# xaynetwork/xaynet

Measured on AMD Instinct MI355X. Metric: masked updates aggregated/sec (25M-param f32 model, PET round: aggregate+all-reduce+unmask), higher is better.
Workload: dtype f32; 1 GPU; model=pet-masked-aggregation-25M, global_batch=1250, seq_len=25000000, parallelism=client-sharded dp1 + rccl all-reduce, mask_config=Prime/F32/B0/M6 (7-byte limbs)

## Files before the change

### xaynet_amd/csrc/gpu/hip_bindings.cpp

```cpp
#include <pybind11/pybind11.h>

#include <pybind11/stl.h>

#include <cmath>
#include <cstring>
#include <stdexcept>
#include <string>
#include <utility>
#include <vector>

#include "kernels.h"

namespace py = pybind11;

struct Limbs {
    xhip_limbs v;
    int n;

    bool is_zero() const { return n == 1 && v.w[0] == 0; }
};

static Limbs parse_limbs(const std::string& dec) {
    if (dec.empty()) throw std::runtime_error("bad decimal");
    Limbs r{{{0, 0, 0, 0, 0}}, 1};
// ... 165 lines not shown

        std::vector<uint32_t> staging(10 * S);
        std::memcpy(staging.data(), seeds.data(), 32 * S);
        std::memcpy(staging.data() + 8 * S, start_words.data(), 8 * S);
        key_.reserve(10 * S, "alloc keys");
        check(hipMemcpy(key_.get(), staging.data(), 40 * S, hipMemcpyHostToDevice), "seed H2D");

        const Plan pl = plan(order, prng_nbytes, len, attempts);
        if (S == 1 || !pl.batchable) {
            uint64_t launched = 0;
            for (uint64_t s = 0; s < S; ++s)
                launched += finish(key_.get() + 8 * s, start_words[s], out_lo + s * seed_stride,
                                   out_hi ? out_hi + s * seed_stride : nullptr, len, order,
                                   prng_nbytes, 0, 0, attempts);
            return launched;
        }

        const uint64_t cand_stride = pl.wgs * 256 * pl.apt;
        const uint32_t counts_stride = uint32_t(pl.wgs);
        cand_lo_.reserve(S * cand_stride, "alloc cand");
        if (order.n == 2) cand_hi_.reserve(S * cand_stride, "alloc cand_hi");
        counts_.reserve(S * counts_stride, "alloc counts");
        total_.reserve(S, "alloc totals");
        check(xhip_k1_expand_batch(
                  key_.get(), reinterpret_cast<const uint64_t*>(key_.get() + 8 * S), uint32_t(S),
                  pl.n_att, pl.wpd, prng_nbytes, order.v.w[0], order.v.w[1], cand_lo_.get(),
                  order.n == 2 ? cand_hi_.get() : nullptr, cand_stride, counts_.get(),
                  counts_stride, total_.get(), pl.apt, out_lo, out_hi, seed_stride, len),
              "k1_expand_batch");
        std::vector<uint64_t> totals(S);
        check(hipMemcpy(totals.data(), total_.get(), 8 * S, hipMemcpyDeviceToHost),
              "totals D2H");
        uint64_t launched = S * pl.n_att;
        for (uint64_t s = 0; s < S; ++s) {
            if (totals[s] >= len) continue;
            launched += finish(key_.get() + 8 * s, start_words[s], out_lo + s * seed_stride,
                               out_hi ? out_hi + s * seed_stride : nullptr, len, order,
                               prng_nbytes, totals[s], pl.n_att, 0) -
                        pl.n_att;
        }
        return launched;
    }

  private:
    uint64_t finish(const uint32_t* key_dev, uint64_t start_word, uint64_t* out_lo,
                    uint64_t* out_hi, uint64_t len, const Limbs& order, int prng_nbytes,
                    uint64_t filled, uint64_t attempt, uint64_t first_attempts) {
        const int L = order.n;
        total_.reserve(1, "alloc total");
        while (filled < len) {
            const Plan pl = plan(order, prng_nbytes, len - filled, first_attempts);
            first_attempts = 0;
            const uint64_t n_att = pl.n_att;
            uint64_t max_wgs = pl.wgs + 2;
            cand_lo_.reserve(L > 2 ? L * n_att : n_att, "alloc cand");
            if (L == 2) cand_hi_.reserve(n_att, "alloc cand_hi");
            uint64_t* cand_hi = L > 2 ? cand_lo_.get() + n_att : cand_hi_.get();
            counts_.reserve(max_wgs, "alloc counts");
            scan_tmp_.reserve(max_wgs / 1024 + 2, "alloc scan tmp");

            uint32_t n_wgs = 0;
            check(xhip_k1_candidates_limbs(key_dev, start_word, attempt, n_att, pl.wpd,
                                           prng_nbytes, order.v, cand_lo_.get(), cand_hi,
                                           counts_.get(), pl.apt, &n_wgs),
                  "k1_candidates");
            check(xhip_k1_scan_hier(counts_.get(), n_wgs, scan_tmp_.get(), total_.get()),
                  "k1_scan");
            check(xhip_k1_scatter_compact_limbs(cand_lo_.get(), cand_hi, counts_.get(),
                                                total_.get(), n_wgs, pl.apt, filled, out_lo,
                                                out_hi, len, order.v),
                  "k1_scatter_compact");
            uint64_t round_accepted = 0;
            check(hipMemcpy(&round_accepted, total_.get(), 8, hipMemcpyDeviceToHost),
                  "total D2H");
            filled += round_accepted;
            if (filled > len) filled = len;
            attempt += n_att;
            if (round_accepted == 0 && n_att > 0 && pl.p <= 0.0)
                throw std::runtime_error("expand: zero acceptance");
        }
        return attempt;
    }

    static constexpr uint64_t kMaxAttemptsPerLaunch = uint64_t(1) << 22;

    DeviceBuffer<uint64_t> cand_lo_;
    DeviceBuffer<uint64_t> cand_hi_;
    DeviceBuffer<uint32_t> counts_;
    DeviceBuffer<uint32_t> scan_tmp_;
    DeviceBuffer<uint64_t> total_;
    DeviceBuffer<uint32_t> key_;
};

PYBIND11_MODULE(_hip, m) {
    m.doc() = "xaynet_amd MI355X (gfx950) kernels: mask expand, aggregate, unmask";
    const auto nogil = py::call_guard<py::gil_scoped_release>();

    m.def("device_count", []() {
        int n = 0;
        hipError_t e = hipGetDeviceCount(&n);
        return e == hipSuccess ? n : 0;
    });
    m.def("synchronize", []() { check(hipDeviceSynchronize(), "sync"); });

    m.def("host_register", [](uintptr_t ptr, size_t size) {
        check(hipHostRegister(reinterpret_cast<void*>(ptr), size, hipHostRegisterDefault),
              "hipHostRegister");
    });
    m.def("host_unregister", [](uintptr_t ptr) {
        check(hipHostUnregister(reinterpret_cast<void*>(ptr)), "hipHostUnregister");
    });

    py::class_<MaskExpander>(m, "MaskExpander")
        .def(py::init<>())
        .def(
            "expand",
            [](MaskExpander& self, const std::string& seed, uintptr_t out_lo, uintptr_t out_hi,
               uint64_t len, const std::string& order, int prng_nbytes, py::object start_word,
               uint64_t seed_stride, uint64_t attempts) {
                std::vector<uint64_t> words;
                if (py::isinstance<py::int_>(start_word))
                    words.push_back(start_word.cast<uint64_t>());
                else
                    words = start_word.cast<std::vector<uint64_t>>();
                py::gil_scoped_release release;
                return self.expand(seed, out_lo, out_hi, len, order, prng_nbytes, words,
                                   seed_stride, attempts);
            },
            py::arg("seed"), py::arg("out_lo"), py::arg("out_hi"), py::arg("len"),
            py::arg("order"), py::arg("prng_nbytes"), py::arg("start_word"), py::kw_only(),
            py::arg("seed_stride") = 0, py::arg("attempts") = 0)
        .def_static("_batch_size", &MaskExpander::batch_size, py::arg("len"), py::arg("order"),
                    py::arg("prng_nbytes"), py::arg("budget_bytes"));

    m.def(
        "aggregate_batch",
        [](uintptr_t acc, uintptr_t updates, uint64_t stride, uint32_t n_updates, uint64_t len,
           int bpn, int ept) {
            check(xhip_k3_aggregate(u64p(acc), u8p(updates), stride, n_updates, len, bpn, ept),
                  "k3_aggregate");
        },
        py::arg("acc"), py::arg("updates"), py::arg("stride"), py::arg("n_updates"),
        py::arg("len"), py::arg("bpn"), py::arg("ept") = 0, nogil);

    m.def(
        "_k3_tile_plan",
        [](uint64_t len, int bpn, uint64_t stride) {
            XhipK3TilePlan p;
            xhip_k3_tile_plan(len, bpn, stride, &p);
            py::dict d;
            d["tile_elems"] = p.tile_elems;
            d["depth"] = p.depth;
            d["waves"] = p.waves;
            d["n_tiles"] = p.n_tiles;
            d["rem_start"] = p.rem_start;
            d["max_byte"] = p.max_byte;
            return d;
        },
        py::arg("len"), py::arg("bpn"), py::arg("stride"));

    m.def(
        "_read_ceiling",
        [](uintptr_t src, uint64_t bytes, bool nontemporal, uintptr_t sink) {
            check(xhip_read_ceiling(u8p(src), bytes, nontemporal,
                                    reinterpret_cast<uint32_t*>(sink)),
                  "read_ceiling");
        },
        py::arg("src"), py::arg("bytes"), py::arg("nontemporal"), py::arg("sink"), nogil);

    m.def(
        "_model_encode",
        [](uintptr_t src, int dtype, uint64_t len, uintptr_t work, uintptr_t out,
           uint64_t out_bytes) -> uint64_t {
            if (dtype < 0 || dtype > 3) throw py::value_error("dtype must be 0..3");
            if (len > (uint64_t(1) << 32))
                throw py::value_error("a model has at most 2^32 weights");
            if (len == 0) return 9;
            py::gil_scoped_release release;
            void* w = reinterpret_cast<void*>(src);
            void* ws = reinterpret_cast<void*>(work);
            check(xhip_k7_model_count(w, dtype, len, ws), "k7_model_count");
            uint64_t words = 0;
            check(hipMemcpy(&words, ws, sizeof words, hipMemcpyDeviceToHost), "k7 total");
            const uint64_t body = 9 + 4 * words;
            if (out_bytes >= 3 + body)
                check(xhip_k7_model_emit(w, dtype, len, ws, u8p(out), out_bytes),
                      "k7_model_emit");
            return body;
        },
        py::arg("src"), py::arg("dtype"), py::arg("len"), py::arg("work"), py::arg("out"),
        py::arg("out_bytes"));

    m.def(
        "_model_plan",
        [](uint64_t len) {
            XhipK7Plan p;
            xhip_k7_plan(len, &p);
            py::dict d;
            d["block_elems"] = p.block_elems;
            d["blocks"] = p.blocks;
            d["scan_levels"] = p.scan_levels;
            d["tile_blocks"] = p.tile_blocks;
            d["tiles"] = p.tiles;
            d["work_bytes"] = p.work_bytes;
            return d;
        },
        py::arg("len"));

    m.def(
        "unmask",
        [](uintptr_t planes, uintptr_t mask_lo, uintptr_t mask_hi, uintptr_t out, uint64_t len,
           int n_planes, const std::string& order, const std::string& exp_shift,
           double n_add_shift, double scalar_sum, int dtype, int digit_bits,
           const std::string& offset, const std::string& divisor) {
            Limbs o = parse_order(order, mask_hi), e = parse_limbs(exp_shift);
            Limbs off = parse_optional(offset), div = parse_optional(divisor);
            check_digit_bits(o, digit_bits);
            if (off.is_zero()) {
                if (o.n > 2)
                    throw py::value_error("orders >= 2^128 are Bmax configs: unmask needs "
                                          "their exact offset");
                if (e.n > 2) throw py::value_error("exp_shift >= 2^128 needs the exact offset");
                if (!div.is_zero()) throw py::value_error("divisor goes with an offset");
            } else if (off.n > o.n) {
                throw py::value_error("the exact offset must be below the order");
            }
            if (div.n > 1) throw py::value_error("divisor must be below 2^64");
            const double scale = double(1.0L / (limbs_to_ld(e) * (long double)scalar_sum));
            check(xhip_k4_unmask_limbs(u64p(planes), u64p(mask_lo), u64p(mask_hi), dtype,
                                       reinterpret_cast<void*>(out), len, n_planes, digit_bits,
                                       o.v, e.v, n_add_shift, scalar_sum, off.v, div.v.w[0],
                                       scale),
                  "k4_unmask");
        },
        py::arg("planes"), py::arg("mask_lo"), py::arg("mask_hi"), py::arg("out"),
        py::arg("len"), py::arg("n_planes"), py::arg("order"), py::arg("exp_shift"),
        py::arg("n_add_shift"), py::arg("scalar_sum"), py::arg("dtype") = 0,
        py::arg("digit_bits") = 32, py::arg("offset") = "", py::arg("divisor") = "", nogil);

    m.def(
        "unmask_values",
        [](uintptr_t vals, uintptr_t mask_lo, uintptr_t mask_hi, uintptr_t out, uint64_t len,
           const std::string& order, const std::string& exp_shift, double n_add_shift,
           double scalar_sum, int dtype, const std::string& offset,
           const std::string& divisor) {
            Limbs o = parse_order(order, mask_hi), e = parse_limbs(exp_shift);
            Limbs off = parse_optional(offset), div = parse_optional(divisor);
            if (o.n > 1 || e.n > 1) throw py::value_error("unmask_values covers u64 orders");
            if (off.n > 1 || div.n > 1)
                throw py::value_error("offset and divisor must be below 2^64");
            if (off.is_zero() && !div.is_zero())
                throw py::value_error("divisor goes with an offset");
            check(xhip_k4_unmask_values(u64p(vals), u64p(mask_lo), dtype,
                                        reinterpret_cast<void*>(out), len, o.v.w[0], e.v.w[0],
                                        n_add_shift, scalar_sum, off.v.w[0], div.v.w[0]),
                  "k4_unmask_values");
        },
        py::arg("vals"), py::arg("mask_lo"), py::arg("mask_hi"), py::arg("out"), py::arg("len"),
        py::arg("order"), py::arg("exp_shift"), py::arg("n_add_shift"), py::arg("scalar_sum"),
        py::arg("dtype") = 0, py::arg("offset") = "", py::arg("divisor") = "", nogil);

    m.def(
        "canonicalize",
        [](uintptr_t planes, uintptr_t out_lo, uintptr_t out_hi, uint64_t len, int n_planes,
           const std::string& order, int digit_bits) {
            Limbs o = parse_order(order, out_hi);
            check_digit_bits(o, digit_bits);
            check(xhip_k2_canonicalize_limbs(u64p(planes), u64p(out_lo), u64p(out_hi), len,
                                             n_planes, digit_bits, o.v),
                  "k2_canonicalize");
        },
        py::arg("planes"), py::arg("out_lo"), py::arg("out_hi"), py::arg("len"),
        py::arg("n_planes"), py::arg("order"), py::arg("digit_bits") = 32, nogil);

    m.def(
        "add_to_planes",
        [](uintptr_t planes, uintptr_t lo, uintptr_t hi, uint64_t len, int n_planes,
           const std::string& order, int digit_bits, uint32_t rows, uint64_t row_stride) {
            Limbs o = parse_order(order, hi);
            check_digit_bits(o, digit_bits);
            if (rows < 1 || rows > XHIP_K1_MAX_BATCH)
                throw py::value_error("rows must be in 1..65535");
            if (rows > 1 && (row_stride == 0 || row_stride < len))
                throw py::value_error("several rows need row_stride, the u64 elements between "
                                      "them (at least len)");
            check(xhip_add_rows_to_planes_limbs(u64p(planes), u64p(lo), u64p(hi), len, n_planes,
                                                digit_bits, o.v, rows, row_stride),
                  "add_to_planes");
        },
        py::arg("planes"), py::arg("lo"), py::arg("hi"), py::arg("len"), py::arg("n_planes"),
        py::arg("order"), py::arg("digit_bits") = 32, py::kw_only(), py::arg("rows") = 1,
        py::arg("row_stride") = 0, nogil);

    m.def(
        "recode_planes",
        [](uintptr_t acc, uintptr_t out, uint64_t len, int n_digits, const std::string& order,
           int k, int digit_bits) {
            Limbs o = parse_limbs(order);
            if (o.n == 1) throw py::value_error("recode_planes covers wide (>= 2^64) orders");
            check(xhip_k2_recode_planes_limbs(u64p(acc), u64p(out), len, n_digits, o.v, k,
                                              digit_bits),
                  "k2_recode_planes");
        },
        py::arg("acc"), py::arg("out"), py::arg("len"), py::arg("n_digits"), py::arg("order"),
        py::arg("k"), py::arg("digit_bits"), nogil);

// ... 94 lines not shown
```

### xaynet_amd/csrc/gpu/kernels.h

```cpp
#pragma once

#include <hip/hip_runtime.h>

#include <cstdint>

#include "limbs.h"

extern "C" {

hipError_t xhip_k1_candidates(const uint32_t* key8_dev, uint64_t start_word,
                              uint64_t first_attempt, uint64_t n_attempts, int words_per_draw,
                              int nbytes, uint64_t order_lo, uint64_t order_hi,
                              uint64_t* cand_lo, uint64_t* cand_hi, uint32_t* wg_counts,
                              int attempts_per_thread, uint32_t* n_wgs_out);
#define XHIP_K1_SCAN_ONE_WG 2048
#define XHIP_K1_MAX_BATCH 65535
hipError_t xhip_k1_scan_hier(uint32_t* wg_counts, uint32_t n, uint32_t* blk_tmp,
                             uint64_t* total_dev);
hipError_t xhip_k1_scatter_compact(const uint64_t* cand_lo, const uint64_t* cand_hi,
                                   const uint32_t* wg_offsets, const uint64_t* total_dev,
                                   uint32_t n_wgs, int apt, uint64_t out_base, uint64_t* out_lo,
                                   uint64_t* out_hi, uint64_t out_len);
hipError_t xhip_k1_expand_batch(const uint32_t* keys_dev, const uint64_t* start_words_dev,
                                uint32_t n_seeds, uint64_t n_attempts, int words_per_draw,
                                int nbytes, uint64_t order_lo, uint64_t order_hi,
                                uint64_t* cand_lo, uint64_t* cand_hi, uint64_t cand_stride,
                                uint32_t* wg_counts, uint32_t counts_stride,
                                uint64_t* totals_dev, int apt, uint64_t* out_lo,
                                uint64_t* out_hi, uint64_t out_stride, uint64_t out_len);

hipError_t xhip_k3_aggregate(uint64_t* acc, const uint8_t* updates, uint64_t stride,
                             uint32_t n_updates, uint64_t len, int bpn, int ept);

struct XhipK3TilePlan {
    uint32_t tile_elems, depth, waves;
    uint64_t n_tiles, rem_start;
    int64_t max_byte;
};
void xhip_k3_tile_plan(uint64_t len, int bpn, uint64_t stride, XhipK3TilePlan* plan);

hipError_t xhip_read_ceiling(const uint8_t* src, uint64_t bytes, bool nontemporal,
                             uint32_t* sink);

hipError_t xhip_k4_unmask(const uint64_t* planes, const uint64_t* mask_lo,
                          const uint64_t* mask_hi, int dtype, void* out, uint64_t len,
                          int n_planes, int digit_bits, uint64_t order_lo, uint64_t order_hi,
                          uint64_t exp_lo, uint64_t exp_hi, double n_add_shift,
                          double scalar_sum);
hipError_t xhip_k4_unmask_values(const uint64_t* vals, const uint64_t* mask, int dtype,
                                 void* out, uint64_t len, uint64_t order, uint64_t exp_shift,
                                 double n_add_shift, double scalar_sum, uint64_t offset,
                                 uint64_t divisor);
hipError_t xhip_k2_canonicalize(const uint64_t* planes, uint64_t* out_lo, uint64_t* out_hi,
                                uint64_t len, int n_planes, int digit_bits, uint64_t order_lo,
                                uint64_t order_hi);
hipError_t xhip_add_to_planes(uint64_t* planes, const uint64_t* lo, const uint64_t* hi,
                              uint64_t len, int n_planes, int digit_bits);
hipError_t xhip_k2_recode_planes(const uint64_t* acc, uint64_t* out, uint64_t len, int n_digits,
                                 uint64_t order_lo, uint64_t order_hi, int k, int digit_bits);
hipError_t xhip_k2_mod_add(uint64_t* a_lo, uint64_t* a_hi, const uint64_t* b_lo,
                           const uint64_t* b_hi, uint64_t len, uint64_t order_lo,
                           uint64_t order_hi);

hipError_t xhip_k5_mask_pack(const uint64_t* mask_lo, const uint64_t* mask_hi, uint8_t* out,
                             uint64_t len, int bpn, uint64_t order_lo, uint64_t order_hi,
                             uint64_t participant, double scalar, double add_shift,
                             uint64_t exp_lo, uint64_t exp_hi);
hipError_t xhip_k5_mask_weights(const void* w, int dtype, const uint64_t* mask_lo,
                                const uint64_t* mask_hi, uint8_t* out, uint64_t len, int bpn,
                                uint64_t order_lo, uint64_t order_hi, double scalar,
                                double add_shift, uint64_t exp_lo, uint64_t exp_hi);

hipError_t xhip_k6_unpack(const uint8_t* in, uint64_t* out_lo, uint64_t* out_hi, uint64_t len,
                          int bpn);
hipError_t xhip_k6_pack(const uint64_t* in_lo, const uint64_t* in_hi, uint8_t* out, uint64_t len,
                        int bpn);

#define XHIP_K7_SCAN_ONE_WG 4096
struct XhipK7Plan {
    uint32_t block_elems, scan_levels, tile_blocks;
    uint64_t blocks, tiles, work_bytes;
};
void xhip_k7_plan(uint64_t len, XhipK7Plan* plan);
hipError_t xhip_k7_model_count(const void* w, int dtype, uint64_t len, void* work);
hipError_t xhip_k7_model_emit(const void* w, int dtype, uint64_t len, const void* work,
                              uint8_t* out, uint64_t out_bytes);

hipError_t xhip_k1_candidates_limbs(const uint32_t* key8_dev, uint64_t start_word,
                                    uint64_t first_attempt, uint64_t n_attempts,
                                    int words_per_draw, int nbytes, xhip_limbs order,
                                    uint64_t* cand_lo, uint64_t* cand_hi, uint32_t* wg_counts,
                                    int attempts_per_thread, uint32_t* n_wgs_out);
hipError_t xhip_k1_scatter_compact_limbs(const uint64_t* cand_lo, const uint64_t* cand_hi,
                                         const uint32_t* wg_offsets, const uint64_t* total_dev,
                                         uint32_t n_wgs, int apt, uint64_t out_base,
                                         uint64_t* out_lo, uint64_t* out_hi, uint64_t out_len,
                                         xhip_limbs order);
hipError_t xhip_k4_unmask_limbs(const uint64_t* planes, const uint64_t* mask_lo,
                                const uint64_t* mask_hi, int dtype, void* out, uint64_t len,
                                int n_planes, int digit_bits, xhip_limbs order,
                                xhip_limbs exp_shift, double n_add_shift, double scalar_sum,
                                xhip_limbs offset, uint64_t divisor, double scale);
hipError_t xhip_k2_canonicalize_limbs(const uint64_t* planes, uint64_t* out_lo,
                                      uint64_t* out_hi, uint64_t len, int n_planes,
                                      int digit_bits, xhip_limbs order);
hipError_t xhip_add_to_planes_limbs(uint64_t* planes, const uint64_t* lo, const uint64_t* hi,
                                    uint64_t len, int n_planes, int digit_bits,
                                    xhip_limbs order);
hipError_t xhip_add_rows_to_planes_limbs(uint64_t* planes, const uint64_t* lo,
                                         const uint64_t* hi, uint64_t len, int n_planes,
                                         int digit_bits, xhip_limbs order, uint32_t rows,
                                         uint64_t row_stride);
hipError_t xhip_k2_recode_planes_limbs(const uint64_t* acc, uint64_t* out, uint64_t len,
                                       int n_digits, xhip_limbs order, int k, int digit_bits);
hipError_t xhip_k2_mod_add_limbs(uint64_t* a_lo, uint64_t* a_hi, const uint64_t* b_lo,
                                 const uint64_t* b_hi, uint64_t len, xhip_limbs order);
hipError_t xhip_k5_mask_weights_limbs(const void* w, int dtype, const uint64_t* mask_lo,
                                      const uint64_t* mask_hi, uint8_t* out, uint64_t len,
                                      int bpn, xhip_limbs order, double scalar, double add_shift,
                                      xhip_limbs exp_shift, xhip_limbs offset);
hipError_t xhip_k5_mask_weights_exact_limbs(const void* w, int dtype, const uint64_t* mask_lo,
                                            const uint64_t* mask_hi, uint8_t* out, uint64_t len,
                                            int bpn, xhip_limbs order, xhip_limbs add_shift,
                                            xhip_limbs exp_shift, uint64_t p, uint64_t q);
hipError_t xhip_k6_unpack_limbs(const uint8_t* in, uint64_t* out_lo, uint64_t* out_hi,
                                uint64_t len, int bpn, xhip_limbs order);
hipError_t xhip_k6_pack_limbs(const uint64_t* in_lo, const uint64_t* in_hi, uint8_t* out,
                              uint64_t len, int bpn, xhip_limbs order);

}
```

### xaynet_amd/csrc/gpu/kernels.hip

```cpp
#include "kernels.h"
#include "mask_quant.h"
#include "model_codec.h"
#include "u192.h"

#include <algorithm>

#define WAVE 64


#define QR(a, b, c, d)                              \
    a += b; d ^= a; d = (d << 16) | (d >> 16);      \
    c += d; b ^= c; b = (b << 12) | (b >> 20);      \
    a += b; d ^= a; d = (d << 8) | (d >> 24);       \
    c += d; b ^= c; b = (b << 7) | (b >> 25)

__device__ void chacha20_block_dev(const uint32_t key[8], uint64_t counter, uint32_t out[16]) {
    uint32_t s[16];
    s[0] = 0x61707865u; s[1] = 0x3320646eu; s[2] = 0x79622d32u; s[3] = 0x6b206574u;
#pragma unroll
    for (int i = 0; i < 8; ++i) s[4 + i] = key[i];
    s[12] = uint32_t(counter);
    s[13] = uint32_t(counter >> 32);
    s[14] = 0;
    s[15] = 0;
// ... 316 lines not shown
            if (v < valid_vec) {
                uint64_t x = __builtin_nontemporal_load(&src[v]);
                lds[2 * v] = uint32_t(x);
                lds[2 * v + 1] = uint32_t(x >> 32);
            }
        }
        __syncthreads();
#pragma unroll
        for (int k = 0; k < EPT; ++k) {
            int e = t + k * TPB;
#pragma unroll
            for (int d = 0; d < NDIG; ++d) {
                int byte0 = e * BPN + 4 * d;
                int nb = (BPN - 4 * d) >= 4 ? 4 : (BPN - 4 * d);
                int wi = byte0 >> 2, sh = (byte0 & 3) * 8;
                uint32_t lo = lds[wi] >> sh;
                uint32_t hi = sh ? (lds[wi + 1] << (32 - sh)) : 0;
                uint32_t val = lo | hi;
                if (nb < 4) val &= (1u << (8 * nb)) - 1;
                racc[k][d] += uint64_t(val);
            }
        }
    }

#pragma unroll
    for (int d = 0; d < NDIG; ++d)
#pragma unroll
        for (int k = 0; k < EPT; ++k) {
            int e = t + k * TPB;
            if (e < nelem_tile) acc[uint64_t(d) * len + tile0 + e] += racc[k][d];
        }
}

typedef uint32_t u32x4 __attribute__((ext_vector_type(4)));

template <int BPN, int T, int D, int WAVES, int AUX>
__global__ __launch_bounds__(WAVES * 64) void k3_aggregate_tile(
    uint64_t* __restrict__ acc, const uint8_t* __restrict__ updates, uint64_t stride,
    uint32_t n_updates, uint64_t len, uint32_t n_tiles) {
    constexpr int NDIG = (BPN + 3) / 4;
    constexpr int NW = (BPN + 6) / 4;
    constexpr int TILE_BYTES = 64 * T * BPN;
    constexpr int PIECES = TILE_BYTES / 1024;
    constexpr int SLOT_WORDS = TILE_BYTES / 4 + 4;
    static_assert(TILE_BYTES % 1024 == 0, "a tile is whole 1-KiB pieces");
    static_assert(D >= 2 && PIECES * (D - 1) <= 63, "vmcnt is a 6-bit count");
    static_assert(AUX == 0 || AUX == 2, "default or nontemporal");
    __shared__ __attribute__((aligned(16))) uint32_t ring[WAVES * D * SLOT_WORDS];

    const uint64_t rem_start = uint64_t(n_tiles) * (64 * T);
    const bool has_rem = rem_start < len;
    if (has_rem && blockIdx.x == 0) {
        constexpr int KR = (T + WAVES - 1) / WAVES;
        uint64_t rr[KR][NDIG];
#pragma unroll
        for (int k = 0; k < KR; ++k)
#pragma unroll
            for (int d = 0; d < NDIG; ++d) rr[k][d] = 0;
        const uint64_t b0 = (rem_start + threadIdx.x) * BPN;
        const uint32_t sh = uint32_t(b0) & 3;
        for (uint32_t u = 0; u < n_updates; ++u) {
            const uint32_t* r =
                reinterpret_cast<const uint32_t*>(updates + uint64_t(u) * stride) + (b0 >> 2);
#pragma unroll
            for (int k = 0; k < KR; ++k) {
                if (rem_start + threadIdx.x + k * (64 * WAVES) >= len) continue;
                uint32_t w[NW];
#pragma unroll
                for (int j = 0; j < NW; ++j) w[j] = r[k * (16 * WAVES * BPN) + j];
#pragma unroll
                for (int d = 0; d < NDIG; ++d) {
                    const int nb = (BPN - 4 * d) >= 4 ? 4 : (BPN - 4 * d);
                    uint32_t val =
                        __builtin_amdgcn_alignbyte(d + 1 < NW ? w[d + 1] : 0u, w[d], sh);
                    if (nb < 4) val &= (1u << (8 * nb)) - 1;
                    rr[k][d] += uint64_t(val);
                }
            }
        }
#pragma unroll
        for (int k = 0; k < KR; ++k) {
            const uint64_t e = rem_start + threadIdx.x + k * (64 * WAVES);
            if (e >= len) continue;
#pragma unroll
            for (int d = 0; d < NDIG; ++d) acc[uint64_t(d) * len + e] += rr[k][d];
        }
        return;
    }

    const uint32_t lane = threadIdx.x & 63;
    const uint32_t wave = __builtin_amdgcn_readfirstlane(threadIdx.x >> 6);
    const uint32_t tile = (blockIdx.x - uint32_t(has_rem)) * WAVES + wave;
    if (tile >= n_tiles) return;

    uint32_t* const wring = ring + wave * (D * SLOT_WORDS);
    const uint8_t* const src = updates + uint64_t(tile) * TILE_BYTES + lane * 16;
    const uint32_t rword = (lane * BPN) >> 2, rsh = (lane * BPN) & 3;

    uint64_t racc[T][NDIG];
#pragma unroll
    for (int k = 0; k < T; ++k)
#pragma unroll
        for (int d = 0; d < NDIG; ++d) racc[k][d] = 0;

    auto issue = [&](uint32_t u, uint32_t slot) {
        const uint8_t* g = src + uint64_t(u) * stride;
        uint32_t* l = wring + slot * SLOT_WORDS;
#pragma unroll
        for (int p = 0; p < PIECES; ++p) {
            auto gp = (const __attribute__((address_space(1))) void*)(g + p * 1024);
            auto lp = (__attribute__((address_space(3))) void*)(l + p * 256);
            if constexpr (AUX == 0)
                __builtin_amdgcn_global_load_lds(gp, lp, 16, 0, 0);
            else
                __builtin_amdgcn_global_load_lds(gp, lp, 16, 0, 2);
        }
    };
    auto consume = [&](uint32_t slot) {
        const uint32_t* r = wring + slot * SLOT_WORDS + rword;
#pragma unroll
        for (int k = 0; k < T; ++k) {
            uint32_t w[NW];
#pragma unroll
            for (int j = 0; j < NW; ++j) w[j] = r[k * 16 * BPN + j];
#pragma unroll
            for (int d = 0; d < NDIG; ++d) {
                const int nb = (BPN - 4 * d) >= 4 ? 4 : (BPN - 4 * d);
                uint32_t val = __builtin_amdgcn_alignbyte(d + 1 < NW ? w[d + 1] : 0u, w[d], rsh);
                if (nb < 4) val &= (1u << (8 * nb)) - 1;
                racc[k][d] += uint64_t(val);
            }
        }
    };
    auto next = [](uint32_t slot) { return slot + 1 == D ? 0u : slot + 1; };

    uint32_t wslot = 0, rslot = 0, u = 0;
    for (; u < n_updates && u < D - 1; ++u) {
        issue(u, wslot);
        wslot = next(wslot);
    }
    for (u = 0; u + (D - 1) < n_updates; ++u) {
        asm volatile("s_waitcnt lgkmcnt(0)" ::: "memory");
        issue(u + (D - 1), wslot);
        wslot = next(wslot);
        asm volatile("s_waitcnt vmcnt(%0)" ::"n"(PIECES * (D - 1)) : "memory");
        consume(rslot);
        rslot = next(rslot);
    }
    asm volatile("s_waitcnt vmcnt(0)" ::: "memory");
    for (; u < n_updates; ++u) {
        consume(rslot);
        rslot = next(rslot);
    }

    const uint64_t e0 = uint64_t(tile) * (64 * T) + lane;
#pragma unroll
    for (int d = 0; d < NDIG; ++d)
#pragma unroll
        for (int k = 0; k < T; ++k) acc[uint64_t(d) * len + e0 + 64 * k] += racc[k][d];
}

template <bool NT>
__global__ void k_read_ceiling(const u32x4* __restrict__ src, uint64_t n_vec,
                               uint32_t* __restrict__ sink) {
    uint64_t i0 = uint64_t(blockIdx.x) * 2048 + threadIdx.x;
    u32x4 x = {0, 0, 0, 0};
    if (uint64_t(blockIdx.x) * 2048 + 2048 <= n_vec) {
        u32x4 v[8];
#pragma unroll
        for (int k = 0; k < 8; ++k)
            v[k] = NT ? __builtin_nontemporal_load(&src[i0 + k * 256]) : src[i0 + k * 256];
#pragma unroll
        for (int k = 0; k < 8; ++k) x ^= v[k];
    } else {
        for (int k = 0; k < 8; ++k) {
            uint64_t i = i0 + k * 256;
            if (i < n_vec) x ^= NT ? __builtin_nontemporal_load(&src[i]) : src[i];
        }
    }
    uint32_t r = x.x ^ x.y ^ x.z ^ x.w;
    if (r == 0x9e3779b9u && (x.x + x.y) == 0x7f4a7c15u) sink[0] = r;
}

template <typename OUT, bool TRUNC>
__global__ void k4_unmask(
    const uint64_t* __restrict__ acc,
    const uint64_t* __restrict__ mask,
    OUT* __restrict__ out, uint64_t len, int n_digits,
    uint64_t order, uint64_t exp_shift, double n_add_shift, double scalar_sum) {
    uint64_t i = uint64_t(blockIdx.x) * blockDim.x + threadIdx.x;
    if (i >= len) return;
    unsigned __int128 v = 0;
    for (int d = n_digits - 1; d >= 0; --d) v = (v << 32) + acc[uint64_t(d) * len + i];
    uint64_t m = uint64_t(v % order);
    uint64_t t = m >= mask[i] ? m - mask[i] : m + order - mask[i];
    double y = double(t / exp_shift) + double(t % exp_shift) / double(exp_shift);
    double r = (y - n_add_shift) / scalar_sum;
    if constexpr (TRUNC)
        out[i] = OUT(trunc(r));
    else
        out[i] = OUT(r);
}

template <typename OUT, bool TRUNC>
__global__ void k4_unmask_values(
    const uint64_t* __restrict__ vals, const uint64_t* __restrict__ mask,
    OUT* __restrict__ out, uint64_t len,
    uint64_t order, uint64_t exp_shift, double n_add_shift, double scalar_sum) {
    uint64_t i = uint64_t(blockIdx.x) * blockDim.x + threadIdx.x;
    if (i >= len) return;
    uint64_t m = vals[i] % order;
    uint64_t t = m >= mask[i] ? m - mask[i] : m + order - mask[i];
    double y = double(t / exp_shift) + double(t % exp_shift) / double(exp_shift);
    double r = (y - n_add_shift) / scalar_sum;
    if constexpr (TRUNC)
        out[i] = OUT(trunc(r));
    else
        out[i] = OUT(r);
}

extern "C" __global__ void k2_canonicalize(
    const uint64_t* __restrict__ acc, uint64_t* __restrict__ out, uint64_t len, int n_digits,
    uint64_t order) {
    uint64_t i = uint64_t(blockIdx.x) * blockDim.x + threadIdx.x;
    if (i >= len) return;
    unsigned __int128 v = 0;
    for (int d = n_digits - 1; d >= 0; --d) v = (v << 32) + acc[uint64_t(d) * len + i];
    out[i] = uint64_t(v % order);
}

extern "C" __global__ void k2_mod_add_u64(
    uint64_t* __restrict__ a, const uint64_t* __restrict__ b, uint64_t len, uint64_t order) {
    uint64_t i = uint64_t(blockIdx.x) * blockDim.x + threadIdx.x;
    if (i >= len) return;
    unsigned __int128 s = (unsigned __int128)a[i] + b[i];
    a[i] = uint64_t(s >= order ? s - order : s);
}

__device__ __forceinline__ uint64_t splitmix64(uint64_t x) {
    x += 0x9e3779b97f4a7c15ULL;
    x = (x ^ (x >> 30)) * 0xbf58476d1ce4e5b9ULL;
    x = (x ^ (x >> 27)) * 0x94d049bb133111ebULL;
    return x ^ (x >> 31);
}

extern "C" __global__ void k5_mask_pack(
    const uint64_t* __restrict__ mask,
    uint8_t* __restrict__ out,
    uint64_t len, int bpn, uint64_t order,
    uint64_t participant, double scalar, double add_shift, double exp_shift_d,
    uint64_t exp_shift) {
    uint64_t i = uint64_t(blockIdx.x) * blockDim.x + threadIdx.x;
    if (i >= len) return;
    uint64_t h = splitmix64(participant * 0x100000001b3ULL + i);
    double w = double(int64_t(h >> 11)) * (2.0 / 9007199254740992.0) - 1.0;
    double scaled = scalar * w;
    if (scaled > add_shift) scaled = add_shift;
    if (scaled < -add_shift) scaled = -add_shift;
    double q = (scaled + add_shift) * exp_shift_d;
    uint64_t shifted = uint64_t(q);
    unsigned __int128 s = (unsigned __int128)shifted + mask[i];
    uint64_t masked = uint64_t(s >= order ? s - order : s);
    uint8_t* p = out + i * bpn;
    for (int b = 0; b < bpn; ++b) p[b] = uint8_t(masked >> (8 * b));
}

extern "C" __global__ void k6_unpack_u64(
    const uint8_t* __restrict__ in, uint64_t* __restrict__ out, uint64_t len, int bpn) {
    uint64_t i = uint64_t(blockIdx.x) * blockDim.x + threadIdx.x;
    if (i >= len) return;
    const uint8_t* p = in + i * bpn;
    uint64_t v = 0;
    for (int b = 0; b < bpn; ++b) v |= uint64_t(p[b]) << (8 * b);
    out[i] = v;
}

extern "C" __global__ void k6_pack_u64(
    const uint64_t* __restrict__ in, uint8_t* __restrict__ out, uint64_t len, int bpn) {
    uint64_t i = uint64_t(blockIdx.x) * blockDim.x + threadIdx.x;
    if (i >= len) return;
    uint64_t v = in[i];
    uint8_t* p = out + i * bpn;
    for (int b = 0; b < bpn; ++b) p[b] = uint8_t(v >> (8 * b));
}

extern "C" __global__ void k_add_u64_to_planes(
    uint64_t* __restrict__ acc, const uint64_t* __restrict__ vals, uint64_t len, int n_digits) {
    uint64_t i = uint64_t(blockIdx.x) * blockDim.x + threadIdx.x;
    if (i >= len) return;
    uint64_t v = vals[i];
    for (int d = 0; d < n_digits; ++d) acc[uint64_t(d) * len + i] += (v >> (32 * d)) & 0xffffffffULL;
}

extern "C" __global__ void k_add_rows_u64_to_planes(
    uint64_t* __restrict__ acc, const uint64_t* __restrict__ vals, uint64_t row_stride,
    uint32_t rows, uint64_t len, int n_digits) {
    uint64_t i = uint64_t(blockIdx.x) * blockDim.x + threadIdx.x;
    if (i >= len) return;
    const uint64_t* p = vals + i;
    uint64_t d0 = 0, d1 = 0;
#pragma unroll 4
    for (uint32_t r = 0; r < rows; ++r) {
        uint64_t v = p[uint64_t(r) * row_stride];
        d0 += v & 0xffffffffULL;
        d1 += v >> 32;
    }
// ... 497 lines not shown
    __shared__ uint32_t wave_tot[K7_BLOCK / WAVE];
    const uint64_t i = uint64_t(blockIdx.x) * K7_BLOCK + threadIdx.x;
    mc_value v = mc_value{0, 0, false};
    uint32_t nw = 0;
    if (i < len) {
        v = mc_decompose(w[i]);
        nw = mc_words(v);
    }
    const uint32_t prefix = block_excl_scan<K7_BLOCK / WAVE>(nw, wave_tot);
    if (i == 0) {
        reinterpret_cast<uint8_t*>(out)[3] = 1;
        out[1] = uint32_t(len);
        out[2] = uint32_t(len >> 32);
    }
    const uint64_t at = 3 + bases[blockIdx.x >> shift] +
                        (in_tile ? in_tile[blockIdx.x] : 0u) + prefix;
    if (i < len && at + nw <= out_words) mc_write(v, out + at);
}


static inline uint32_t ceil_div_u32(uint64_t a, uint64_t b) { return uint32_t((a + b - 1) / b); }

template <typename K, typename... Args>
static hipError_t launch_1d(K kernel, uint64_t len, Args... args) {
    if (len == 0) return hipSuccess;
    kernel<<<dim3(ceil_div_u32(len, 256)), dim3(256), 0, 0>>>(args...);
    return hipGetLastError();
}

template <typename T, bool TRUNC>
struct DType {
    using type = T;
    static constexpr bool trunc = TRUNC;
};

template <typename F>
static hipError_t dispatch_dtype(int dtype, F f) {
    switch (dtype) {
        case 0: return f(DType<float, false>{});
        case 1: return f(DType<double, false>{});
        case 2: return f(DType<int32_t, true>{});
        case 3: return f(DType<int64_t, true>{});
        default: return hipErrorInvalidValue;
    }
}


hipError_t xhip_k1_candidates(const uint32_t* key8_dev, uint64_t start_word,
                              uint64_t first_attempt, uint64_t n_attempts, int words_per_draw,
                              int nbytes, uint64_t order_lo, uint64_t order_hi,
                              uint64_t* cand_lo, uint64_t* cand_hi, uint32_t* wg_counts,
                              int attempts_per_thread, uint32_t* n_wgs_out) {
    uint32_t wgs = ceil_div_u32(n_attempts, uint64_t(K1_LDS_THREADS) * attempts_per_thread);
    *n_wgs_out = wgs;
    if (order_hi != 0)
        hipLaunchKernelGGL(k1_candidates_lds_u128, dim3(wgs), dim3(K1_LDS_THREADS), 0, 0,
                           key8_dev, start_word, first_attempt, n_attempts, words_per_draw,
                           nbytes, order_lo, order_hi, cand_lo, cand_hi, wg_counts,
                           attempts_per_thread);
    else
        hipLaunchKernelGGL(k1_candidates_lds, dim3(wgs), dim3(K1_LDS_THREADS), 0, 0, key8_dev,
                           start_word, first_attempt, n_attempts, words_per_draw, nbytes,
                           order_lo, cand_lo, wg_counts, attempts_per_thread);
    return hipGetLastError();
}

hipError_t xhip_k1_scan_hier(uint32_t* wg_counts, uint32_t n, uint32_t* blk_tmp,
                             uint64_t* total_dev) {
    if (n <= XHIP_K1_SCAN_ONE_WG) {
        hipLaunchKernelGGL(k1_scan, dim3(1), dim3(1024), 0, 0, wg_counts, n, total_dev);
        return hipGetLastError();
    }
    uint32_t nblk = (n + 1023) / 1024;
    hipLaunchKernelGGL(k1_scan_blocks, dim3(nblk), dim3(256), 0, 0, wg_counts, n, blk_tmp);
    hipLaunchKernelGGL(k1_scan, dim3(1), dim3(1024), 0, 0, blk_tmp, nblk, total_dev);
    hipLaunchKernelGGL(k1_scan_addbase, dim3(nblk), dim3(256), 0, 0, wg_counts, n, blk_tmp);
    return hipGetLastError();
}

hipError_t xhip_k1_scatter_compact(const uint64_t* cand_lo, const uint64_t* cand_hi,
                                   const uint32_t* wg_offsets, const uint64_t* total_dev,
                                   uint32_t n_wgs, int apt, uint64_t out_base, uint64_t* out_lo,
                                   uint64_t* out_hi, uint64_t out_len) {
    if (n_wgs == 0) return hipSuccess;
    if (out_hi)
        hipLaunchKernelGGL(k1_scatter_compact_u128, dim3(n_wgs), dim3(256), 0, 0, cand_lo,
                           cand_hi, wg_offsets, total_dev, n_wgs, 256 * apt, out_base, out_lo,
                           out_hi, out_len);
    else
        hipLaunchKernelGGL(k1_scatter_compact, dim3(n_wgs), dim3(256), 0, 0, cand_lo,
                           wg_offsets, total_dev, n_wgs, 256 * apt, out_base, out_lo, out_len);
    return hipGetLastError();
}

hipError_t xhip_k1_expand_batch(const uint32_t* keys_dev, const uint64_t* start_words_dev,
                                uint32_t n_seeds, uint64_t n_attempts, int words_per_draw,
                                int nbytes, uint64_t order_lo, uint64_t order_hi,
                                uint64_t* cand_lo, uint64_t* cand_hi, uint64_t cand_stride,
                                uint32_t* wg_counts, uint32_t counts_stride,
                                uint64_t* totals_dev, int apt, uint64_t* out_lo,
                                uint64_t* out_hi, uint64_t out_stride, uint64_t out_len) {
    if (apt < 1 || n_attempts == 0) return hipErrorInvalidValue;
    const uint64_t cap = uint64_t(K1_LDS_THREADS) * apt;
    const uint64_t wgs64 = (n_attempts + cap - 1) / cap;
    if (n_seeds < 1 || n_seeds > XHIP_K1_MAX_BATCH || wgs64 > XHIP_K1_SCAN_ONE_WG ||
        counts_stride < wgs64 || cand_stride < wgs64 * cap ||
        (order_hi != 0) != (out_hi != nullptr) || (order_hi != 0 && !cand_hi))
        return hipErrorInvalidValue;
    const uint32_t wgs = uint32_t(wgs64);
    const dim3 grid(wgs, n_seeds);
    if (order_hi != 0)
        hipLaunchKernelGGL(k1_candidates_lds_u128_batch, grid, dim3(K1_LDS_THREADS), 0, 0,
                           keys_dev, start_words_dev, n_attempts, words_per_draw, nbytes,
                           order_lo, order_hi, cand_lo, cand_hi, cand_stride, wg_counts,
                           counts_stride, apt);
    else
        hipLaunchKernelGGL(k1_candidates_lds_batch, grid, dim3(K1_LDS_THREADS), 0, 0, keys_dev,
                           start_words_dev, n_attempts, words_per_draw, nbytes, order_lo,
                           cand_lo, cand_stride, wg_counts, counts_stride, apt);
    hipLaunchKernelGGL(k1_scan_seg, dim3(n_seeds), dim3(1024), 0, 0, wg_counts, counts_stride,
                       wgs, totals_dev);
    hipLaunchKernelGGL(order_hi != 0 ? k1_scatter_compact_batch<true>
                                     : k1_scatter_compact_batch<false>,
                       grid, dim3(256), 0, 0, cand_lo, cand_hi, cand_stride, wg_counts,
                       counts_stride, totals_dev, wgs, int(cap), out_lo, out_hi, out_stride,
                       out_len);
    return hipGetLastError();
}


#define K3_TILE_CONFIGS(X)                                                                      \
    X(3, 16, 3, 4)                                                                              \
    X(7, 16, 3, 4)                                                                              \
    X(10, 8, 3, 4)                                                                              \
    X(18, 8, 2, 4)                                                                              \
    X(40, 4, 2, 4)

void xhip_k3_tile_plan(uint64_t len, int bpn, uint64_t stride, XhipK3TilePlan* plan) {
    *plan = XhipK3TilePlan{0, 0, 0, 0, 0, -1};
    uint32_t t = 0, d = 0, waves = 0;
#define K3_TILE_ROW(BPN, T, D, WAVES)                                                           \
    if (bpn == BPN) t = T, d = D, waves = WAVES;
    K3_TILE_CONFIGS(K3_TILE_ROW)
#undef K3_TILE_ROW
    if (t == 0 || stride % 16 != 0 || stride < 16 || len > (stride - 16) / uint64_t(bpn)) return;
    plan->tile_elems = 64 * t;
    plan->depth = d;
    plan->waves = waves;
    plan->n_tiles = std::min<uint64_t>(len / plan->tile_elems, 0x7fffffffu);
    plan->rem_start = plan->n_tiles * plan->tile_elems;
    if (plan->n_tiles) plan->max_byte = int64_t(plan->rem_start * uint64_t(bpn)) - 1;
}

hipError_t xhip_k3_aggregate(uint64_t* acc, const uint8_t* updates, uint64_t stride,
                             uint32_t n_updates, uint64_t len, int bpn, int ept) {
    uint32_t threads = 256;
    if (ept <= 0 && bpn == 7) ept = 401;
    if (ept == 401 || ept == 402) {
        XhipK3TilePlan plan;
        xhip_k3_tile_plan(len, bpn, stride, &plan);
        if (plan.n_tiles && reinterpret_cast<uintptr_t>(updates) % 16 == 0) {
            const uint64_t blocks_extra = plan.rem_start < len ? 1 : 0;
#define K3_TILE_CASE(BPN, T, D, WAVES)                                                          \
    case BPN: {                                                                                 \
        dim3 grid(ceil_div_u32(plan.n_tiles, WAVES) + blocks_extra), block(WAVES * 64);         \
        if (ept == 401)                                                                         \
            hipLaunchKernelGGL((k3_aggregate_tile<BPN, T, D, WAVES, 2>), grid, block, 0, 0,     \
                               acc, updates, stride, n_updates, len, uint32_t(plan.n_tiles));   \
        else                                                                                    \
            hipLaunchKernelGGL((k3_aggregate_tile<BPN, T, D, WAVES, 0>), grid, block, 0, 0,     \
                               acc, updates, stride, n_updates, len, uint32_t(plan.n_tiles));   \
        return hipGetLastError();                                                               \
    }
            switch (bpn) {
                K3_TILE_CONFIGS(K3_TILE_CASE)
                default:;
            }
#undef K3_TILE_CASE
        }
        ept = 0;
    }
#define K3_LAUNCH(BPN, EPT)                                                                     \
    {                                                                                           \
        uint32_t wgs = ceil_div_u32((len + EPT - 1) / EPT, threads);                            \
        hipLaunchKernelGGL((k3_aggregate<BPN, EPT>), dim3(wgs), dim3(threads), 0, 0, acc,       \
                           updates, stride, n_updates, len);                                    \
    }
#define K3_CASE(BPN, DEFEPT, ALT1, ALT2)                                                        \
    case BPN:                                                                                   \
        if (ept == ALT1)                                                                        \
            K3_LAUNCH(BPN, ALT1)                                                                \
        else if (ept == ALT2)                                                                   \
            K3_LAUNCH(BPN, ALT2)                                                                \
        else                                                                                    \
            K3_LAUNCH(BPN, DEFEPT)                                                              \
        break;
    if (ept == 201 || ept == 202) {
        uintptr_t base = reinterpret_cast<uintptr_t>(updates);
        if ((base % 16) == 0 && (stride % 16) == 0) {
#define K3_LDS_CASE(BPN)                                                                        \
    case BPN: {                                                                                 \
        if (ept == 201) {                                                                       \
            uint32_t wgs = ceil_div_u32((len + 2047) / 2048, 1);                                \
            hipLaunchKernelGGL((k3_aggregate_lds<BPN, 2048>), dim3(wgs), dim3(256), 0, 0, acc,  \
                               updates, stride, n_updates, len);                                \
        } else {                                                                                \
            uint32_t wgs = ceil_div_u32((len + 4095) / 4096, 1);                                \
            hipLaunchKernelGGL((k3_aggregate_lds<BPN, 4096>), dim3(wgs), dim3(256), 0, 0, acc,  \
                               updates, stride, n_updates, len);                                \
        }                                                                                       \
        return hipGetLastError();                                                               \
    }
            switch (bpn) {
                K3_LDS_CASE(1)
                K3_LDS_CASE(2)
                K3_LDS_CASE(3)
                K3_LDS_CASE(4)
                K3_LDS_CASE(5)
                K3_LDS_CASE(6)
                K3_LDS_CASE(7)
                K3_LDS_CASE(8)
                default:;
            }
#undef K3_LDS_CASE
        }
        ept = 0;
    }
    switch (bpn) {
        K3_CASE(1, 16, 32, 16)
        K3_CASE(2, 8, 16, 8)
        K3_CASE(3, 16, 16, 16)
        K3_CASE(4, 4, 8, 16)
        K3_CASE(5, 16, 16, 16)
        K3_CASE(6, 8, 8, 8)
        K3_CASE(7, 4, 8, 16)
        K3_CASE(8, 4, 2, 8)
        K3_CASE(9, 4, 4, 4)
        K3_CASE(10, 2, 4, 8)
        K3_CASE(11, 4, 4, 4)
        K3_CASE(12, 2, 4, 2)
        K3_CASE(13, 4, 4, 4)
        K3_CASE(14, 2, 4, 2)
        K3_CASE(15, 4, 4, 4)
        K3_CASE(16, 2, 4, 1)
        K3_CASE(18, 2, 2, 2)
        K3_CASE(37, 4, 4, 4)
        K3_CASE(38, 2, 2, 2)
        K3_CASE(39, 4, 4, 4)
        K3_CASE(40, 2, 1, 2)
        default:
            return hipErrorInvalidValue;
    }
#undef K3_CASE
#undef K3_LAUNCH
    return hipGetLastError();
}

hipError_t xhip_read_ceiling(const uint8_t* src, uint64_t bytes, bool nontemporal,
                             uint32_t* sink) {
    if (reinterpret_cast<uintptr_t>(src) % 16 || bytes % 16) return hipErrorInvalidValue;
    const uint64_t n_vec = bytes / 16;
    if (n_vec == 0 || n_vec / 2048 >= 0x7fffffffu) return hipErrorInvalidValue;
    dim3 grid(uint32_t((n_vec + 2047) / 2048)), block(256);
    if (nontemporal)
        hipLaunchKernelGGL(k_read_ceiling<true>, grid, block, 0, 0,
                           reinterpret_cast<const u32x4*>(src), n_vec, sink);
    else
        hipLaunchKernelGGL(k_read_ceiling<false>, grid, block, 0, 0,
                           reinterpret_cast<const u32x4*>(src), n_vec, sink);
    return hipGetLastError();
}


static bool bad_planes(bool wide, int n_planes, int digit_bits) {
    if (n_planes < 1) return true;
    return wide ? digit_bits < 1 || digit_bits > 63 : digit_bits != 32;
}

static bool outside_window(int n_limbs, int n_planes, int digit_bits) {
    return int64_t(n_planes - 1) * digit_bits + 64 > 64 * (n_limbs + 1) - 1;
}

static bool bad_read_planes(bool wide, int n_planes, int digit_bits) {
    return bad_planes(wide, n_planes, digit_bits) ||
           (wide && outside_window(2, n_planes, digit_bits));
}

static double u128_to_double(uint64_t lo, uint64_t hi) {
    return double(((unsigned __int128)hi << 64) | lo);
}

hipError_t xhip_k4_unmask(const uint64_t* planes, const uint64_t* mask_lo,
                          const uint64_t* mask_hi, int dtype, void* out, uint64_t len,
                          int n_planes, int digit_bits, uint64_t order_lo, uint64_t order_hi,
                          uint64_t exp_lo, uint64_t exp_hi, double n_add_shift,
                          double scalar_sum) {
    const bool wide = order_hi != 0;
    if (bad_read_planes(wide, n_planes, digit_bits) || (!wide && exp_hi))
        return hipErrorInvalidValue;
    return dispatch_dtype(dtype, [&](auto t) {
        using OUT = typename decltype(t)::type;
        constexpr bool TRUNC = decltype(t)::trunc;
        OUT* o = static_cast<OUT*>(out);
        if (!wide)
            return launch_1d(k4_unmask<OUT, TRUNC>, len, planes, mask_lo, o, len, n_planes,
                             order_lo, exp_lo, n_add_shift, scalar_sum);
        return launch_1d(digit_bits == 32 ? k4_unmask_u128<OUT, TRUNC, 32>
                                          : k4_unmask_u128<OUT, TRUNC, 0>,
                         len, planes, mask_lo, mask_hi, o, len, n_planes, digit_bits, order_lo,
                         order_hi, exp_lo, exp_hi, n_add_shift, scalar_sum);
    });
}

hipError_t xhip_k4_unmask_values(const uint64_t* vals, const uint64_t* mask, int dtype,
                                 void* out, uint64_t len, uint64_t order, uint64_t exp_shift,
                                 double n_add_shift, double scalar_sum, uint64_t offset,
                                 uint64_t divisor) {
    return dispatch_dtype(dtype, [&](auto t) {
        using OUT = typename decltype(t)::type;
        constexpr bool TRUNC = decltype(t)::trunc;
        if (offset) {
            if constexpr (TRUNC) {
                if (!exp_shift || offset >= order) return hipErrorInvalidValue;
                return launch_1d(k4_unmask_offset<OUT, TRUNC, 1>, len, vals, mask, int64_t(0),
                                 static_cast<OUT*>(out), len, 1, 32,
                                 xhip_limbs{{order, 0, 0, 0, 0}},
                                 xhip_limbs{{offset, 0, 0, 0, 0}}, exp_shift, divisor,
                                 scalar_sum, 0.0);
            } else {
                return hipErrorInvalidValue;
            }
// ... 411 lines not shown
```

Measured before the change: 34790 updates/s.

## Add warp-specialized loader kernel for k3 aggregation with LDS ring pipeline

Adds a k3_aggregate_loader kernel in which one producer wave issues async global_load_lds copies into a shared-memory ring of depth D. CONS consumer waves then unpack the bytes into limb digits and accumulate them, with the two sides synchronised by barriers and vmcnt waits. For 7-byte limbs the default path switches from the existing tile kernel to this loader kernel. The aim is to decouple memory streaming from the unpack ALU work so HBM reads stay in flight. In exchange, one wave per block does no arithmetic, and barrier coupling may serialise progress.

Result: faster. 37020 updates/s, median of 6 (+6.4%).

```diff
diff --git a/xaynet_amd/csrc/gpu/hip_bindings.cpp b/xaynet_amd/csrc/gpu/hip_bindings.cpp
--- a/xaynet_amd/csrc/gpu/hip_bindings.cpp
+++ b/xaynet_amd/csrc/gpu/hip_bindings.cpp
@@ -341,6 +341,23 @@
             d["tile_elems"] = p.tile_elems;
             d["depth"] = p.depth;
             d["waves"] = p.waves;
+            d["n_tiles"] = p.n_tiles;
+            d["rem_start"] = p.rem_start;
+            d["max_byte"] = p.max_byte;
+            return d;
+        },
+        py::arg("len"), py::arg("bpn"), py::arg("stride"));
+
+    m.def(
+        "_k3_loader_plan",
+        [](uint64_t len, int bpn, uint64_t stride) {
+            XhipK3LoaderPlan p;
+            xhip_k3_loader_plan(len, bpn, stride, &p);
+            py::dict d;
+            d["consumers"] = p.consumers;
+            d["depth"] = p.depth;
+            d["tile_blocks"] = p.tile_blocks;
+            d["has_remainder"] = bool(p.has_remainder);
             d["n_tiles"] = p.n_tiles;
             d["rem_start"] = p.rem_start;
             d["max_byte"] = p.max_byte;
diff --git a/xaynet_amd/csrc/gpu/kernels.h b/xaynet_amd/csrc/gpu/kernels.h
--- a/xaynet_amd/csrc/gpu/kernels.h
+++ b/xaynet_amd/csrc/gpu/kernels.h
@@ -38,6 +38,13 @@
     int64_t max_byte;
 };
 void xhip_k3_tile_plan(uint64_t len, int bpn, uint64_t stride, XhipK3TilePlan* plan);
+
+struct XhipK3LoaderPlan {
+    uint32_t consumers, depth, tile_blocks, has_remainder;
+    uint64_t n_tiles, rem_start;
+    int64_t max_byte;
+};
+void xhip_k3_loader_plan(uint64_t len, int bpn, uint64_t stride, XhipK3LoaderPlan* plan);
 
 hipError_t xhip_read_ceiling(const uint8_t* src, uint64_t bytes, bool nontemporal,
                              uint32_t* sink);
diff --git a/xaynet_amd/csrc/gpu/kernels.hip b/xaynet_amd/csrc/gpu/kernels.hip
--- a/xaynet_amd/csrc/gpu/kernels.hip
+++ b/xaynet_amd/csrc/gpu/kernels.hip
@@ -492,6 +492,156 @@
         consume(rslot);
         rslot = next(rslot);
     }
+
+    const uint64_t e0 = uint64_t(tile) * (64 * T) + lane;
+#pragma unroll
+    for (int d = 0; d < NDIG; ++d)
+#pragma unroll
+        for (int k = 0; k < T; ++k) acc[uint64_t(d) * len + e0 + 64 * k] += racc[k][d];
+}
+
+template <int BPN, int T, int D, int CONS, int AUX>
+__global__ __launch_bounds__((1 + CONS) * 64) void k3_aggregate_loader(
+    uint64_t* __restrict__ acc, const uint8_t* __restrict__ updates, uint64_t stride,
+    uint32_t n_updates, uint64_t len, uint32_t n_tiles) {
+    constexpr int NDIG = (BPN + 3) / 4;
+    constexpr int NW = (BPN + 6) / 4;
+    constexpr int NWAVES = 1 + CONS;
+    constexpr int TILE_BYTES = 64 * T * BPN;
+    constexpr int PIECES = TILE_BYTES / 1024;
+    constexpr int PB = CONS * PIECES;
+    constexpr int SLOT_WORDS = TILE_BYTES / 4 + 4;
+    static_assert(TILE_BYTES % 1024 == 0, "a tile is whole 1-KiB pieces");
+    static_assert(D >= 2 && PB * (D - 2) <= 63, "vmcnt is a 6-bit count");
+    static_assert(AUX == 0 || AUX == 2, "default or nontemporal");
+    __shared__ __attribute__((aligned(16))) uint32_t ring[D * CONS * SLOT_WORDS];
+
+    const uint64_t rem_start = uint64_t(n_tiles) * (64 * T);
+    const bool has_rem = rem_start < len;
+    if (has_rem && blockIdx.x == 0) {
+        constexpr int KR = (T + NWAVES - 1) / NWAVES;
+        uint64_t rr[KR][NDIG];
+#pragma unroll
+        for (int k = 0; k < KR; ++k)
+#pragma unroll
+            for (int d = 0; d < NDIG; ++d) rr[k][d] = 0;
+        const uint64_t b0 = (rem_start + threadIdx.x) * BPN;
+        const uint32_t sh = uint32_t(b0) & 3;
+        for (uint32_t u = 0; u < n_updates; ++u) {
+            const uint32_t* r =
+                reinterpret_cast<const uint32_t*>(updates + uint64_t(u) * stride) + (b0 >> 2);
+#pragma unroll
+            for (int k = 0; k < KR; ++k) {
+                if (rem_start + threadIdx.x + k * (64 * NWAVES) >= len) continue;
+                uint32_t w[NW];
+#pragma unroll
+                for (int j = 0; j < NW; ++j) w[j] = r[k * (16 * NWAVES * BPN) + j];
+#pragma unroll
+                for (int d = 0; d < NDIG; ++d) {
+                    const int nb = (BPN - 4 * d) >= 4 ? 4 : (BPN - 4 * d);
+                    uint32_t val =
+                        __builtin_amdgcn_alignbyte(d + 1 < NW ? w[d + 1] : 0u, w[d], sh);
+                    if (nb < 4) val &= (1u << (8 * nb)) - 1;
+                    rr[k][d] += uint64_t(val);
+                }
+            }
+        }
+#pragma unroll
+        for (int k = 0; k < KR; ++k) {
+            const uint64_t e = rem_start + threadIdx.x + k * (64 * NWAVES);
+            if (e >= len) continue;
+#pragma unroll
+            for (int d = 0; d < NDIG; ++d) acc[uint64_t(d) * len + e] += rr[k][d];
+        }
+        return;
+    }
+
+    const uint32_t lane = threadIdx.x & 63;
+    const uint32_t wave = __builtin_amdgcn_readfirstlane(threadIdx.x >> 6);
+    const uint32_t tile0 = (blockIdx.x - uint32_t(has_rem)) * CONS;
+    auto next = [](uint32_t slot) { return slot + 1 == D ? 0u : slot + 1; };
+
+    if (wave == 0) {
+        const uint8_t* src[CONS];
+#pragma unroll
+        for (int c = 0; c < CONS; ++c) {
+            const uint32_t t = tile0 + c < n_tiles ? tile0 + c : n_tiles - 1;
+            src[c] = updates + uint64_t(t) * TILE_BYTES + lane * 16;
+        }
+        auto issue = [&](uint32_t u, uint32_t slot) {
+            uint32_t* l = ring + slot * (CONS * SLOT_WORDS);
+#pragma unroll
+            for (int c = 0; c < CONS; ++c) {
+                const uint8_t* g = src[c] + uint64_t(u) * stride;
+#pragma unroll
+                for (int p = 0; p < PIECES; ++p) {
+                    auto gp = (const __attribute__((address_space(1))) void*)(g + p * 1024);
+                    auto lp =
+                        (__attribute__((address_space(3))) void*)(l + c * SLOT_WORDS + p * 256);
+                    if constexpr (AUX == 0)
+                        __builtin_amdgcn_global_load_lds(gp, lp, 16, 0, 0);
+                    else
+                        __builtin_amdgcn_global_load_lds(gp, lp, 16, 0, 2);
+                }
+            }
+        };
+        uint32_t wslot = 0, k = 0;
+        for (; k < n_updates && k < D - 1; ++k) {
+            issue(k, wslot);
+            wslot = next(wslot);
+        }
+        for (k = 0; k + (D - 1) < n_updates; ++k) {
+            asm volatile("s_waitcnt vmcnt(%0)" ::"n"(PB * (D - 2)) : "memory");
+            __builtin_amdgcn_s_barrier();
+            asm volatile("" ::: "memory");
+            issue(k + (D - 1), wslot);
+            wslot = next(wslot);
+        }
+        for (; k < n_updates; ++k) {
+            asm volatile("s_waitcnt vmcnt(0)" ::: "memory");
+            __builtin_amdgcn_s_barrier();
+        }
+        return;
+    }
+
+    const uint32_t c = wave - 1;
+    const uint32_t tile = tile0 + c;
+    const bool live = tile < n_tiles;
+    const uint32_t rword = (lane * BPN) >> 2, rsh = (lane * BPN) & 3;
+    const uint32_t* const cring = ring + c * SLOT_WORDS + rword;
+
+    uint64_t racc[T][NDIG];
+#pragma unroll
+    for (int k = 0; k < T; ++k)
+#pragma unroll
+        for (int d = 0; d < NDIG; ++d) racc[k][d] = 0;
+
+    auto consume = [&](uint32_t slot) {
+        const uint32_t* r = cring + slot * (CONS * SLOT_WORDS);
+#pragma unroll
+        for (int k = 0; k < T; ++k) {
+            uint32_t w[NW];
+#pragma unroll
+            for (int j = 0; j < NW; ++j) w[j] = r[k * 16 * BPN + j];
+#pragma unroll
+            for (int d = 0; d < NDIG; ++d) {
+                const int nb = (BPN - 4 * d) >= 4 ? 4 : (BPN - 4 * d);
+                uint32_t val = __builtin_amdgcn_alignbyte(d + 1 < NW ? w[d + 1] : 0u, w[d], rsh);
+                if (nb < 4) val &= (1u << (8 * nb)) - 1;
+                racc[k][d] += uint64_t(val);
+            }
+        }
+    };
+
+    uint32_t rslot = 0;
+    for (uint32_t k = 0; k < n_updates; ++k) {
+        __builtin_amdgcn_s_barrier();
+        asm volatile("" ::: "memory");
+        if (live) consume(rslot);
+        rslot = next(rslot);
+        asm volatile("s_waitcnt lgkmcnt(0)" ::: "memory");
+    }
+    if (!live) return;
 
     const uint64_t e0 = uint64_t(tile) * (64 * T) + lane;
 #pragma unroll
@@ -1295,10 +1445,34 @@
     if (plan->n_tiles) plan->max_byte = int64_t(plan->rem_start * uint64_t(bpn)) - 1;
 }
 
+#define K3_LOADER_CONFIGS(X)                                                                    \
+    X(3, 16, 3, 4)                                                                              \
+    X(7, 16, 2, 8)                                                                              \
+    X(10, 8, 3, 4)
+
+void xhip_k3_loader_plan(uint64_t len, int bpn, uint64_t stride, XhipK3LoaderPlan* plan) {
+    *plan = XhipK3LoaderPlan{0, 0, 0, 0, 0, 0, -1};
+    uint32_t d = 0, cons = 0;
+#define K3_LOADER_ROW(BPN, T, D, CONS)                                                          \
+    if (bpn == BPN) d = D, cons = CONS;
+    K3_LOADER_CONFIGS(K3_LOADER_ROW)
+#undef K3_LOADER_ROW
+    XhipK3TilePlan tiles;
+    xhip_k3_tile_plan(len, bpn, stride, &tiles);
+    if (cons == 0 || tiles.n_tiles == 0) return;
+    plan->consumers = cons;
+    plan->depth = d;
+    plan->tile_blocks = ceil_div_u32(tiles.n_tiles, cons);
+    plan->has_remainder = tiles.rem_start < len ? 1 : 0;
+    plan->n_tiles = tiles.n_tiles;
+    plan->rem_start = tiles.rem_start;
+    plan->max_byte = tiles.max_byte;
+}
+
 hipError_t xhip_k3_aggregate(uint64_t* acc, const uint8_t* updates, uint64_t stride,
                              uint32_t n_updates, uint64_t len, int bpn, int ept) {
     uint32_t threads = 256;
-    if (ept <= 0 && bpn == 7) ept = 401;
+    if (ept <= 0 && bpn == 7) ept = 411;
     if (ept == 401 || ept == 402) {
         XhipK3TilePlan plan;
         xhip_k3_tile_plan(len, bpn, stride, &plan);
@@ -1320,6 +1494,29 @@
                 default:;
             }
 #undef K3_TILE_CASE
+        }
+        ept = 0;
+    }
+    if (ept == 411 || ept == 412) {
+        XhipK3LoaderPlan lp;
+        xhip_k3_loader_plan(len, bpn, stride, &lp);
+        if (lp.tile_blocks && reinterpret_cast<uintptr_t>(updates) % 16 == 0) {
+#define K3_LOADER_CASE(BPN, T, D, CONS)                                                         \
+    case BPN: {                                                                                 \
+        dim3 grid(lp.tile_blocks + lp.has_remainder), block((1 + CONS) * 64);                   \
+        if (ept == 411)                                                                         \
+            hipLaunchKernelGGL((k3_aggregate_loader<BPN, T, D, CONS, 2>), grid, block, 0, 0,    \
+                               acc, updates, stride, n_updates, len, uint32_t(lp.n_tiles));     \
+        else                                                                                    \
+            hipLaunchKernelGGL((k3_aggregate_loader<BPN, T, D, CONS, 0>), grid, block, 0, 0,    \
+                               acc, updates, stride, n_updates, len, uint32_t(lp.n_tiles));     \
+        return hipGetLastError();                                                               \
+    }
+            switch (bpn) {
+                K3_LOADER_CONFIGS(K3_LOADER_CASE)
+                default:;
+            }
+#undef K3_LOADER_CASE
         }
         ept = 0;
     }
```
